# MMAThijssen/catfish

Measured on AMD Instinct MI355X. Metric: signal samples/s classified, higher is better.
Workload: dtype f32

## Files before the change

catfish_amd/csrc/catfish_hip.hip:

```cpp
#include <hip/hip_runtime.h>
#include <stdint.h>
#include <string.h>
#include <stdio.h>
#include <vector>
#include <string>
#include <cmath>
#include <mutex>
#include <set>
#include <functional>

#include "../../include/catfish_hip.h"

typedef float f32x4 __attribute__((ext_vector_type(4)));
typedef float f32x2 __attribute__((ext_vector_type(2)));

#define CF_T 35
#define CF_H 64
#define CF_C 32
#define CF_TILE 16

#define MFMA16(a, b, c) __builtin_amdgcn_mfma_f32_16x16x4f32((a), (b), (c), 0, 0, 0)

#ifndef CF_ABLATE
#define CF_ABLATE 0
#endif
#ifndef CF_PREFETCH
#define CF_PREFETCH 1
#endif

__device__ __forceinline__ float cf_sigmoid(float x) {
    return __builtin_amdgcn_rcpf(1.0f + __expf(-x));
}
__device__ __forceinline__ float cf_tanh(float x) {
    return fmaf(-2.0f, __builtin_amdgcn_rcpf(1.0f + __expf(2.0f * x)), 1.0f);
}
#define CF_GATE_SCALE (-1.4426950408889634)
#define CF_CAND_SCALE (2.8853900817779268)
__device__ __forceinline__ float cf_sigmoid_pre(float a) {
    return __builtin_amdgcn_rcpf(1.0f + __builtin_amdgcn_exp2f(a));
}
__device__ __forceinline__ float cf_tanh_pre(float a) {
    return fmaf(-2.0f, __builtin_amdgcn_rcpf(1.0f + __builtin_amdgcn_exp2f(a)), 1.0f);
}
__device__ __forceinline__ f32x2 cf_sigmoid_pre2(f32x2 a) {
    f32x2 e = {__builtin_amdgcn_exp2f(a.x), __builtin_amdgcn_exp2f(a.y)};
    e = e + (f32x2){1.0f, 1.0f};
    return (f32x2){__builtin_amdgcn_rcpf(e.x), __builtin_amdgcn_rcpf(e.y)};
}
__device__ __forceinline__ f32x2 cf_tanh_pre2(f32x2 a) {
    return __builtin_elementwise_fma((f32x2){-2.0f, -2.0f}, cf_sigmoid_pre2(a), (f32x2){1.0f, 1.0f});
}
template <typename T>
struct far_lds {
    static constexpr int N64K = 65536 / sizeof(T);
    const T *b0, *b1, *b2;
    __device__ __forceinline__ explicit far_lds(const T* base) {
        int o1 = N64K, o2 = 2 * N64K;
        asm volatile("" : "+v"(o1), "+v"(o2));
        b0 = base; b1 = base + o1; b2 = base + o2;
    }
    __device__ __forceinline__ const T& operator[](int e) const { return e < N64K ? b0[e] : (e < 2 * N64K ? b1[e - N64K] : b2[e - 2 * N64K]); }
};
__device__ __forceinline__ f32x4 cf_sigmoid_pre4(f32x4 a) {
    f32x4 e = {__builtin_amdgcn_exp2f(a.x), __builtin_amdgcn_exp2f(a.y), __builtin_amdgcn_exp2f(a.z), __builtin_amdgcn_exp2f(a.w)};
    e = e + (f32x4){1.0f, 1.0f, 1.0f, 1.0f};
    return (f32x4){__builtin_amdgcn_rcpf(e.x), __builtin_amdgcn_rcpf(e.y), __builtin_amdgcn_rcpf(e.z), __builtin_amdgcn_rcpf(e.w)};
}
__device__ __forceinline__ f32x4 cf_tanh_pre4(f32x4 a) {
    return __builtin_elementwise_fma((f32x4){-2.0f, -2.0f, -2.0f, -2.0f}, cf_sigmoid_pre4(a), (f32x4){1.0f, 1.0f, 1.0f, 1.0f});
}
struct cf_dropout {
    float keep_prob = 1.f;
    uint32_t seed = 0;
    int32_t layer = 0;
    const double* step = nullptr;
};
__device__ __forceinline__ uint32_t cf_fmix32(uint32_t v) {
    v ^= v >> 16; v *= 0x85ebca6bu; v ^= v >> 13; v *= 0xc2b2ae35u; v ^= v >> 16;
    return v;
}
__device__ __forceinline__ uint32_t cf_drop_key(const cf_dropout& d) {
    const uint32_t st = d.step ? (uint32_t)(long long)d.step[0] : 0u;
    return cf_fmix32(d.seed ^ cf_fmix32(0x9E3779B9u * (uint32_t)(d.layer + 1) + st * 0x85ebca6bu));
}
__device__ __forceinline__ f32x4 cf_drop_scale4(uint32_t key, float keep_prob, int64_t idx4) {
    const uint32_t thresh = (uint32_t)fminf(keep_prob * 4294967296.0f, 4294967040.0f);
    const float inv = 1.0f / keep_prob;
    const uint64_t e = (uint64_t)idx4 * 4u;
    const uint32_t base = (uint32_t)e ^ ((uint32_t)(e >> 32) * 0x9E3779B9u);
    f32x4 o;
    o.x = cf_fmix32((base + 0u) ^ key) < thresh ? inv : 0.f;
    o.y = cf_fmix32((base + 1u) ^ key) < thresh ? inv : 0.f;
    o.z = cf_fmix32((base + 2u) ^ key) < thresh ? inv : 0.f;
    o.w = cf_fmix32((base + 3u) ^ key) < thresh ? inv : 0.f;
    return o;
}

__device__ __forceinline__ f32x4 relu4(f32x4 v) {
    f32x4 o;
    o.x = fmaxf(v.x, 0.f); o.y = fmaxf(v.y, 0.f); o.z = fmaxf(v.z, 0.f); o.w = fmaxf(v.w, 0.f);
    return o;
}

__host__ __device__ constexpr int gru_x_floats(int cin) { return (cin / 4) * 3 * 256; }
__host__ __device__ constexpr int gru_hg_floats() { return 16 * 2 * 256; }
__host__ __device__ constexpr int gru_hc_floats() { return 16 * 256; }
__host__ __device__ constexpr int gru_bias_off(int cin) { return gru_x_floats(cin) + gru_hg_floats() + gru_hc_floats(); }
__host__ __device__ constexpr int gru_dense_off(int cin) { return gru_bias_off(cin) + 192; }
__host__ __device__ constexpr int gru_pack_floats(int cin) { return gru_dense_off(cin) + 64; }
#include "tuned_launch.hpp"

__host__ __device__ constexpr int res_units(bool first) { return first ? 4 : 6; }
__host__ __device__ constexpr int res_vecs(bool first) { return first ? 6 : 4; }
__host__ __device__ constexpr int res_pack_floats(bool first) { return res_units(first) * 1024 + res_vecs(first) * 32; }

__host__ __device__ constexpr int frag_feature(int ks, int q) { return 16 * (ks >> 2) + 4 * q + (ks & 3); }

__device__ __forceinline__ void unit_mma(const float* __restrict__ unit, int lane, const f32x4 (&in)[2], f32x4 (&acc)[2]) {
    const f32x2* u2 = reinterpret_cast<const f32x2*>(unit) + lane;
#pragma unroll
    for (int ks = 0; ks < 8; ++ks) {
        const f32x2 a = u2[ks * 64];
        const float b = in[ks >> 2][ks & 3];
        acc[0] = MFMA16(a.x, b, acc[0]);
        acc[1] = MFMA16(a.y, b, acc[1]);
    }
}

template <bool FIRST>
__global__ __launch_bounds__(256) void res_block_kernel(const float* __restrict__ wpack,
                                                        const float* __restrict__ x_nat,
                                                        const f32x4* __restrict__ x_frag,
                                                        f32x4* __restrict__ y_frag,
                                                        int64_t n_windows, int n_tiles, int t_chunks) {
    extern __shared__ __attribute__((aligned(16))) float lds[];
    constexpr int PACK = res_pack_floats(FIRST);
    constexpr int VEC0 = res_units(FIRST) * 1024;
    {
        const f32x4* src = reinterpret_cast<const f32x4*>(wpack);
        f32x4* dst = reinterpret_cast<f32x4*>(lds);
        for (int i = threadIdx.x; i < PACK / 4; i += blockDim.x) dst[i] = src[i];
    }
    __syncthreads();
    const int lane = threadIdx.x & 63;
    const int wave = __builtin_amdgcn_readfirstlane(threadIdx.x >> 6);
    const int q = lane >> 4;
    const int waves_per_block = blockDim.x >> 6;
    float* xs = lds + PACK + wave * (CF_TILE * CF_T);

    auto vec = [&](int v, int mo) -> f32x4 {
        return *reinterpret_cast<const f32x4*>(lds + VEC0 + v * 32 + mo * 16 + q * 4);
    };

    const int chunk_len = (CF_T + t_chunks - 1) / t_chunks;
    for (int task = blockIdx.x * waves_per_block + wave; task < n_tiles * t_chunks; task += gridDim.x * waves_per_block) {
        const int tile = task / t_chunks;
        const int p0 = (task - tile * t_chunks) * chunk_len;
        const int p1 = min(p0 + chunk_len, CF_T);
        f32x4 w_sc[2], b_sc[2], w_f[2], b_f[2];
        if constexpr (FIRST) {
            const int64_t base = (int64_t)tile * CF_TILE * CF_T;
            const int64_t limit = n_windows * CF_T;
            for (int i = lane; i < CF_TILE * CF_T; i += 64) xs[i] = (base + i < limit) ? x_nat[base + i] : 0.f;
#pragma unroll
            for (int mo = 0; mo < 2; ++mo) { w_sc[mo] = vec(2, mo); b_sc[mo] = vec(3, mo); w_f[mo] = vec(4, mo); b_f[mo] = vec(5, mo); }
            __builtin_amdgcn_fence(__ATOMIC_RELEASE, "wavefront");
            __builtin_amdgcn_wave_barrier();
            __builtin_amdgcn_fence(__ATOMIC_ACQUIRE, "wavefront");
        }
        f32x4 o1_pp[2] = {{0, 0, 0, 0}, {0, 0, 0, 0}};
        f32x4 o1_p[2] = {{0, 0, 0, 0}, {0, 0, 0, 0}};
        f32x4 sc_p[2] = {{0, 0, 0, 0}, {0, 0, 0, 0}};
        for (int i = p0 > 0 ? p0 - 1 : 0; i <= p1; ++i) {
            f32x4 o1_c[2] = {{0, 0, 0, 0}, {0, 0, 0, 0}};
            f32x4 sc_c[2] = {{0, 0, 0, 0}, {0, 0, 0, 0}};
            if (i < CF_T) {
                if constexpr (FIRST) {
                    const float xv = xs[(lane & 15) * CF_T + i];
#pragma unroll
                    for (int mo = 0; mo < 2; ++mo) {
                        sc_c[mo] = w_sc[mo] * xv + b_sc[mo];
                        o1_c[mo] = relu4(w_f[mo] * xv + b_f[mo]);
                    }
                } else {
                    f32x4 in[2];
                    const f32x4* src = x_frag + ((int64_t)tile * CF_T + i) * 2 * 64 + lane;
                    in[0] = src[0];
                    in[1] = src[64];
                    sc_c[0] = vec(0, 0); sc_c[1] = vec(0, 1);
                    unit_mma(lds + 0 * 1024, lane, in, sc_c);
                    f32x4 acc[2] = {vec(1, 0), vec(1, 1)};
                    unit_mma(lds + 1 * 1024, lane, in, acc);
                    o1_c[0] = relu4(acc[0]); o1_c[1] = relu4(acc[1]);
                }
            }
            if (i >= p0 + 1) {
                constexpr int U3 = FIRST ? 0 : 2;
                constexpr int VB3 = FIRST ? 0 : 2;
                f32x4 acc[2] = {vec(VB3, 0), vec(VB3, 1)};
                unit_mma(lds + (U3 + 0) * 1024, lane, o1_pp, acc);
                unit_mma(lds + (U3 + 1) * 1024, lane, o1_p, acc);
                unit_mma(lds + (U3 + 2) * 1024, lane, o1_c, acc);
                f32x4 o2[2] = {relu4(acc[0]), relu4(acc[1])};
                f32x4 acc3[2] = {vec(VB3 + 1, 0), vec(VB3 + 1, 1)};
                unit_mma(lds + (U3 + 3) * 1024, lane, o2, acc3);
                f32x4* dst = y_frag + ((int64_t)tile * CF_T + (i - 1)) * 2 * 64 + lane;
                dst[0] = relu4(relu4(acc3[0]) + sc_p[0]);
                dst[64] = relu4(relu4(acc3[1]) + sc_p[1]);
            }
#pragma unroll
            for (int mo = 0; mo < 2; ++mo) { o1_pp[mo] = o1_p[mo]; o1_p[mo] = o1_c[mo]; sc_p[mo] = sc_c[mo]; }
        }
        if constexpr (FIRST) __builtin_amdgcn_wave_barrier();
    }
}

template <bool CHUNKED>
__global__ __launch_bounds__(256) void res_stack2_kernel(const float* __restrict__ wpack0, const float* __restrict__ wpack1,
                                                         const float* __restrict__ x_nat,
                                                         f32x4* __restrict__ y_frag,
                                                         f32x4* __restrict__ y0_frag,
                                                         int64_t n_windows, int n_tiles, int t_chunks) {
    extern __shared__ __attribute__((aligned(16))) float lds[];
    constexpr int PACK0 = res_pack_floats(true), PACK1 = res_pack_floats(false);
    constexpr int VEC0 = res_units(true) * 1024, VEC1 = res_units(false) * 1024;
    {
        const f32x4* src0 = reinterpret_cast<const f32x4*>(wpack0);
        const f32x4* src1 = reinterpret_cast<const f32x4*>(wpack1);
        f32x4* dst = reinterpret_cast<f32x4*>(lds);
        for (int i = threadIdx.x; i < PACK0 / 4; i += blockDim.x) dst[i] = src0[i];
        for (int i = threadIdx.x; i < PACK1 / 4; i += blockDim.x) dst[PACK0 / 4 + i] = src1[i];
    }
    __syncthreads();
    const int lane = threadIdx.x & 63;
    const int wave = __builtin_amdgcn_readfirstlane(threadIdx.x >> 6);
    const int q = lane >> 4;
    const int waves_per_block = blockDim.x >> 6;
    const float* w0 = lds;
    const float* w1 = lds + PACK0;
    float* xs = lds + PACK0 + PACK1 + wave * (CF_TILE * CF_T);
    auto vec0 = [&](int v, int mo) -> f32x4 { return *reinterpret_cast<const f32x4*>(w0 + VEC0 + v * 32 + mo * 16 + q * 4); };
    auto vec1 = [&](int v, int mo) -> f32x4 { return *reinterpret_cast<const f32x4*>(w1 + VEC1 + v * 32 + mo * 16 + q * 4); };
    const f32x4 zero = {0, 0, 0, 0};

    if (!CHUNKED) t_chunks = 1;
    const int chunk_len = CHUNKED ? (CF_T + t_chunks - 1) / t_chunks : CF_T;
    for (int task = blockIdx.x * waves_per_block + wave; task < n_tiles * t_chunks; task += gridDim.x * waves_per_block) {
        const int tile = CHUNKED ? task / t_chunks : task;
        const int p0 = CHUNKED ? (task - tile * t_chunks) * chunk_len : 0;
        const int p1 = CHUNKED ? min(p0 + chunk_len, CF_T) : CF_T;
        if (CHUNKED && p0 >= p1) continue;
        {
            const int64_t base = (int64_t)tile * CF_TILE * CF_T;
            const int64_t limit = n_windows * CF_T;
            for (int i = lane; i < CF_TILE * CF_T; i += 64) xs[i] = (base + i < limit) ? x_nat[base + i] : 0.f;
            __builtin_amdgcn_fence(__ATOMIC_RELEASE, "wavefront");
            __builtin_amdgcn_wave_barrier();
            __builtin_amdgcn_fence(__ATOMIC_ACQUIRE, "wavefront");
        }
        f32x4 w_sc[2], b_sc[2], w_f[2], b_f[2];
#pragma unroll
        for (int mo = 0; mo < 2; ++mo) { w_sc[mo] = vec0(2, mo); b_sc[mo] = vec0(3, mo); w_f[mo] = vec0(4, mo); b_f[mo] = vec0(5, mo); }
        f32x4 a_pp[2] = {zero, zero}, a_p[2] = {zero, zero}, a_sp[2] = {zero, zero};
        f32x4 b_pp[2] = {zero, zero}, b_p[2] = {zero, zero}, b_sp[2] = {zero, zero};
        for (int i = p0 > 2 ? p0 - 2 : 0; i <= p1 + 1; ++i) {
            f32x4 a_c[2] = {zero, zero}, a_sc[2] = {zero, zero};
            if (i < CF_T) {
                const float xv = xs[(lane & 15) * CF_T + i];
#pragma unroll
                for (int mo = 0; mo < 2; ++mo) {
                    a_sc[mo] = w_sc[mo] * xv + b_sc[mo];
                    a_c[mo] = relu4(w_f[mo] * xv + b_f[mo]);
                }
            }
            f32x4 y0[2] = {zero, zero};
            const bool have_y0 = i >= 1 && i <= CF_T && i >= p0;
            if (have_y0) {
                f32x4 acc[2] = {vec0(0, 0), vec0(0, 1)};
                unit_mma(w0 + 0 * 1024, lane, a_pp, acc);
                unit_mma(w0 + 1 * 1024, lane, a_p, acc);
                unit_mma(w0 + 2 * 1024, lane, a_c, acc);
                f32x4 o2[2] = {relu4(acc[0]), relu4(acc[1])};
                f32x4 acc3[2] = {vec0(1, 0), vec0(1, 1)};
                unit_mma(w0 + 3 * 1024, lane, o2, acc3);
                y0[0] = relu4(relu4(acc3[0]) + a_sp[0]);
                y0[1] = relu4(relu4(acc3[1]) + a_sp[1]);
                if (CHUNKED && y0_frag && i - 1 >= p0 && i - 1 < p1) {
                    f32x4* d0 = y0_frag + ((int64_t)tile * CF_T + (i - 1)) * 2 * 64 + lane;
                    d0[0] = y0[0];
                    d0[64] = y0[1];
                }
            }
            f32x4 b_c[2] = {zero, zero}, b_sc[2] = {zero, zero};
            if (have_y0) {
                b_sc[0] = vec1(0, 0); b_sc[1] = vec1(0, 1);
                unit_mma(w1 + 0 * 1024, lane, y0, b_sc);
                f32x4 acc[2] = {vec1(1, 0), vec1(1, 1)};
                unit_mma(w1 + 1 * 1024, lane, y0, acc);
                b_c[0] = relu4(acc[0]); b_c[1] = relu4(acc[1]);
            }
            if (i >= 2 && i - 2 >= p0 && i - 2 < p1) {
                f32x4 acc[2] = {vec1(2, 0), vec1(2, 1)};
                unit_mma(w1 + 2 * 1024, lane, b_pp, acc);
                unit_mma(w1 + 3 * 1024, lane, b_p, acc);
                unit_mma(w1 + 4 * 1024, lane, b_c, acc);
                f32x4 o2[2] = {relu4(acc[0]), relu4(acc[1])};
                f32x4 acc3[2] = {vec1(3, 0), vec1(3, 1)};
                unit_mma(w1 + 5 * 1024, lane, o2, acc3);
                f32x4* dst = y_frag + ((int64_t)tile * CF_T + (i - 2)) * 2 * 64 + lane;
                dst[0] = relu4(relu4(acc3[0]) + b_sp[0]);
                dst[64] = relu4(relu4(acc3[1]) + b_sp[1]);
            }
#pragma unroll
            for (int mo = 0; mo < 2; ++mo) {
                a_pp[mo] = a_p[mo]; a_p[mo] = a_c[mo]; a_sp[mo] = a_sc[mo];
                if (i >= 1) { b_pp[mo] = b_p[mo]; b_p[mo] = b_c[mo]; b_sp[mo] = b_sc[mo]; }
            }
        }
        __builtin_amdgcn_wave_barrier();
    }
}

template <int CIN>
__device__ __forceinline__ void gru_stage_weights(float* lds, const float* __restrict__ wpack, int dir) {
    constexpr int PACK = gru_pack_floats(CIN);
    const f32x4* src = reinterpret_cast<const f32x4*>(wpack + (size_t)dir * PACK);
    f32x4* dst = reinterpret_cast<f32x4*>(lds);
    for (int i = threadIdx.x; i < PACK / 4; i += blockDim.x) dst[i] = src[i];
}

#ifndef CF_SCHED_DS_FIRST
#define CF_SCHED_DS_FIRST 1
#endif
#if CF_SCHED_DS_FIRST
#define CF_KSTEP_SCHED(nds, nmfma)                               \
    __builtin_amdgcn_sched_group_barrier(0x100, nds, 0);         \
    __builtin_amdgcn_sched_group_barrier(0x008, nmfma, 0);       \
    __builtin_amdgcn_sched_barrier(0)
#else
#define CF_KSTEP_SCHED(nds, nmfma) __builtin_amdgcn_sched_barrier(0)
#endif
template <int CIN, bool LAST, bool STASH = false, bool SKIP0 = false>
__device__ __forceinline__ void gru_tile(const float* lds, int lane, int dir, int tile, const f32x4* __restrict__ X,
                                         f32x4* __restrict__ Y, float* __restrict__ P, int n_tiles,
                                         f32x4* __restrict__ S = nullptr, f32x4* __restrict__ YD = nullptr, cf_dropout drop = cf_dropout(),
                                         int s_begin = 0, int s_end = CF_T, f32x4* HO = nullptr, bool skip0 = false) {
    const uint32_t drop_key = (STASH && YD) ? cf_drop_key(drop) : 0u;
    constexpr int KGX = CIN / 16;
    constexpr int KSX = CIN / 4;
    constexpr int XN4 = gru_x_floats(CIN) / 4;
    constexpr int HG4 = gru_hg_floats() / 4;
    constexpr int BIAS = gru_bias_off(CIN);
    constexpr int DENSE = gru_dense_off(CIN);
    const int q = lane >> 4;
    const f32x4* WX = reinterpret_cast<const f32x4*>(lds) + lane;
    const far_lds<f32x4> WL(WX);
    const f32x4* B4 = reinterpret_cast<const f32x4*>(lds + BIAS) + q;
    const f32x4* D4 = reinterpret_cast<const f32x4*>(lds + DENSE) + q;
    {
        f32x4 h[4] = {{0, 0, 0, 0}, {0, 0, 0, 0}, {0, 0, 0, 0}, {0, 0, 0, 0}};
        if (s_begin > 0) {
#pragma unroll
            for (int m = 0; m < 4; ++m) h[m] = HO[m * 64 + lane];
        }
        f32x4 xc[KGX];
        {
            const int t0 = dir ? (CF_T - 1 - s_begin) : s_begin;
            const f32x4* src = X + ((int64_t)tile * CF_T + t0) * KGX * 64 + lane;
#pragma unroll
            for (int g = 0; g < KGX; ++g) xc[g] = src[g * 64];
        }
        for (int s = s_begin; s < s_end; ++s) {
            const int t = dir ? (CF_T - 1 - s) : s;
            f32x4 acc[12];
#pragma unroll
            for (int mo = 0; mo < 12; ++mo) acc[mo] = B4[mo * 4];
            constexpr int PF = CF_PREFETCH;
            auto loadA = [&](int p, f32x4 (&d)[3]) {
                if (p < KSX) { d[0] = WL[(p * 3 + 0) * 64]; d[1] = WL[(p * 3 + 1) * 64]; d[2] = WL[(p * 3 + 2) * 64]; }
                else if (p < KSX + 16) { d[0] = WL[XN4 + ((p - KSX) * 2 + 0) * 64]; d[1] = WL[XN4 + ((p - KSX) * 2 + 1) * 64]; }
                else if (p < KSX + 32) { d[0] = WL[XN4 + HG4 + (p - KSX - 16) * 64]; }
            };
            f32x4 ac[3], an[3], a2[3];
            loadA(0, ac);
            if (PF == 2) loadA(1, an);
#pragma unroll
            for (int ks = 0; ks < KSX; ++ks) {
                if (PF == 2) loadA(ks + 2, a2); else loadA(ks + 1, an);
                const float b = xc[ks >> 2][ks & 3];
#pragma unroll
                for (int g = 0; g < 3; ++g) {
                    acc[4 * g + 0] = MFMA16(ac[g].x, b, acc[4 * g + 0]);
                    acc[4 * g + 1] = MFMA16(ac[g].y, b, acc[4 * g + 1]);
                    acc[4 * g + 2] = MFMA16(ac[g].z, b, acc[4 * g + 2]);
                    acc[4 * g + 3] = MFMA16(ac[g].w, b, acc[4 * g + 3]);
                }
                CF_KSTEP_SCHED(3, 12);
#pragma unroll
                for (int g = 0; g < 3; ++g) { ac[g] = an[g]; if (PF == 2) an[g] = a2[g]; }
            }
            {
                int tn = dir ? (t - 1) : (t + 1);
                tn = tn < 0 ? 0 : (tn > CF_T - 1 ? CF_T - 1 : tn);
                const f32x4* src = X + ((int64_t)tile * CF_T + tn) * KGX * 64 + lane;
#pragma unroll
                for (int g = 0; g < KGX; ++g) if (!(CF_ABLATE & 2)) xc[g] = src[g * 64];
            }
            const bool run_h = !SKIP0 || !(skip0 && s == 0);
            if constexpr (SKIP0) {
#pragma unroll
                for (int mo = 0; mo < 12; ++mo) asm volatile("" : "+v"(acc[mo]));
            }
            if (run_h) {
#pragma unroll
            for (int ks = 0; ks < 16; ++ks) {
                if (PF == 2) loadA(KSX + ks + 2, a2); else loadA(KSX + ks + 1, an);
                const float b = h[ks >> 2][ks & 3];
#pragma unroll
                for (int g = 0; g < 2; ++g) {
                    acc[4 * g + 0] = MFMA16(ac[g].x, b, acc[4 * g + 0]);
                    acc[4 * g + 1] = MFMA16(ac[g].y, b, acc[4 * g + 1]);
                    acc[4 * g + 2] = MFMA16(ac[g].z, b, acc[4 * g + 2]);
                    acc[4 * g + 3] = MFMA16(ac[g].w, b, acc[4 * g + 3]);
                }
                CF_KSTEP_SCHED(2, 8);
                ac[0] = an[0]; ac[1] = an[1];
                if (PF == 2) { an[0] = a2[0]; an[1] = a2[1]; }
            }
            f32x4 rh[4];
#pragma unroll
            for (int m = 0; m < 4; ++m) {
                if (CF_ABLATE & 1) { rh[m] = acc[m] * 0.001f; continue; }
                const f32x4 rv = cf_sigmoid_pre4(acc[m]);
                rh[m] = rv * h[m];
                if constexpr (STASH) acc[m] = rv;
            }
#pragma unroll
            for (int ks = 0; ks < 16; ++ks) {
                if (PF == 2) loadA(KSX + 16 + ks + 2, a2); else loadA(KSX + 16 + ks + 1, an);
                const float b = rh[ks >> 2][ks & 3];
                acc[8] = MFMA16(ac[0].x, b, acc[8]);
                acc[9] = MFMA16(ac[0].y, b, acc[9]);
                acc[10] = MFMA16(ac[0].z, b, acc[10]);
                acc[11] = MFMA16(ac[0].w, b, acc[11]);
                CF_KSTEP_SCHED(1, 4);
                ac[0] = an[0];
                if (PF == 2) an[0] = a2[0];
            }
            }
#pragma unroll
            for (int m = 0; m < 4; ++m) {
                if (CF_ABLATE & 1) { h[m] = acc[4 + m] * 0.001f + acc[8 + m] * 0.001f; continue; }
                const f32x4 u = cf_sigmoid_pre4(acc[4 + m]);
                const f32x4 c = cf_tanh_pre4(acc[8 + m]);
                h[m] = __builtin_elementwise_fma(u, h[m] - c, c);
                if constexpr (STASH) { acc[4 + m] = u; acc[8 + m] = c; }
            }
            if constexpr (STASH) {
                f32x4* sdst = S + (((int64_t)tile * CF_T + t) * 2 + dir) * 12 * 64 + lane;
#pragma unroll
                for (int j = 0; j < 12; ++j) sdst[j * 64] = acc[j];
            }
            if constexpr (!LAST) {
                f32x4* dst = Y + (((int64_t)tile * CF_T + t) * 8 + dir * 4) * 64 + lane;
#pragma unroll
                for (int m = 0; m < 4; ++m) if (!(CF_ABLATE & 2) || s == CF_T - 1) dst[m * 64] = h[m];
                if constexpr (STASH) {
                    if (YD) {
                        const int64_t i0 = (((int64_t)tile * CF_T + t) * 8 + dir * 4) * 64 + lane;
#pragma unroll
                        for (int m = 0; m < 4; ++m) YD[i0 + m * 64] = h[m] * cf_drop_scale4(drop_key, drop.keep_prob, i0 + m * 64);
                    }
                }
            } else {
                float pm[4];
#pragma unroll
                for (int m = 0; m < 4; ++m) {
                    const f32x4 wd = D4[m * 4];
                    pm[m] = wd.x * h[m].x;
                    pm[m] = fmaf(wd.y, h[m].y, pm[m]); pm[m] = fmaf(wd.z, h[m].z, pm[m]); pm[m] = fmaf(wd.w, h[m].w, pm[m]);
                }
                float p = ((pm[0] + pm[1]) + pm[2]) + pm[3];
                p += __shfl_xor(p, 16);
                p += __shfl_xor(p, 32);
                if (lane < 16) P[(((int64_t)dir * n_tiles + tile) * CF_T + t) * 16 + lane] = p;
            }
            __builtin_amdgcn_sched_barrier(0);
        }
        if (s_end < CF_T) {
#pragma unroll
            for (int m = 0; m < 4; ++m) HO[m * 64 + lane] = h[m];
        }
    }
}

__device__ __forceinline__ void cf_handoff_publish(unsigned* flag) {
    asm volatile("s_waitcnt vmcnt(0)" ::: "memory");
    __builtin_amdgcn_fence(__ATOMIC_RELEASE, "workgroup");
    asm volatile("s_waitcnt vmcnt(0)" ::: "memory");
    __hip_atomic_store(flag, 1u, __ATOMIC_RELAXED, __HIP_MEMORY_SCOPE_WORKGROUP);
}
__device__ __forceinline__ void cf_handoff_wait(unsigned* flag, int lane, unsigned* err) {
    if (lane == 0) {
        bool ok = false;
        for (int it = 0; it < 1000000 && !ok; ++it) {
            ok = __hip_atomic_load(flag, __ATOMIC_RELAXED, __HIP_MEMORY_SCOPE_WORKGROUP) != 0u;
            if (!ok) __builtin_amdgcn_s_sleep(16);
        }
        if (!ok && err) __hip_atomic_store(err, 1u, __ATOMIC_RELAXED, __HIP_MEMORY_SCOPE_SYSTEM);
    }
    __builtin_amdgcn_fence(__ATOMIC_ACQUIRE, "workgroup");
    asm volatile("s_waitcnt vmcnt(0)" ::: "memory");
}
__device__ __forceinline__ void cf_handoff_publish_agent(unsigned* flag) {
    asm volatile("s_waitcnt vmcnt(0)" ::: "memory");
    __builtin_amdgcn_fence(__ATOMIC_RELEASE, "agent");
    asm volatile("s_waitcnt vmcnt(0)" ::: "memory");
    __hip_atomic_store(flag, 1u, __ATOMIC_RELAXED, __HIP_MEMORY_SCOPE_AGENT);
}
__device__ __forceinline__ void cf_handoff_wait_agent(unsigned* flag, int lane, unsigned* err) {
    if (lane == 0) {
        bool ok = false;
        for (int it = 0; it < 1000000 && !ok; ++it) {
            ok = __hip_atomic_load(flag, __ATOMIC_RELAXED, __HIP_MEMORY_SCOPE_AGENT) != 0u;
            if (!ok) __builtin_amdgcn_s_sleep(16);
        }
        if (!ok && err) __hip_atomic_store(err, 1u, __ATOMIC_RELAXED, __HIP_MEMORY_SCOPE_SYSTEM);
    }
    __builtin_amdgcn_fence(__ATOMIC_ACQUIRE, "agent");
    asm volatile("s_waitcnt vmcnt(0)" ::: "memory");
    if (lane == 0) __hip_atomic_store(flag, 0u, __ATOMIC_RELAXED, __HIP_MEMORY_SCOPE_AGENT);
}


template <int CIN, bool LAST>
__global__ __launch_bounds__(512, 2) void gru_layer_kernel(const float* __restrict__ wpack,
                                                           const f32x4* __restrict__ X,
                                                           f32x4* __restrict__ Y,
                                                           float* __restrict__ P,
                                                           int n_tiles,
                                                           int balance_arg,
                                                           f32x4* hand,
                                                           unsigned* gflags,
                                                           unsigned* err) {
    extern __shared__ __attribute__((aligned(16))) float lds[];
    const int dir = blockIdx.y;
    gru_stage_weights<CIN>(lds, wpack, dir);
    unsigned* flags = reinterpret_cast<unsigned*>(lds + gru_pack_floats(CIN));
    if (threadIdx.x < CF_GRU_MAX_WAVES) flags[threadIdx.x] = 0u;
    __syncthreads();
    const int lane = threadIdx.x & 63;
    const int wave = __builtin_amdgcn_readfirstlane(threadIdx.x >> 6);
    const int nwaves = blockDim.x >> 6;
    const int balance = balance_arg & CF_GRU_SCHED_MASK;
    const bool skip0 = !(balance_arg & CF_GRU_RUN_ZERO_PRODUCTS);
    int t0 = (int)((int64_t)blockIdx.x * n_tiles / gridDim.x);
    const int t1 = (int)((int64_t)(blockIdx.x + 1) * n_tiles / gridDim.x);
    cf_gru_share sh;
    int n_pieces;
    if (balance == 2) {
        sh = cf_gru_balanced_share(n_tiles, (int)gridDim.x * nwaves, (int)blockIdx.x * nwaves + wave, CF_T);
        n_pieces = (sh.head_end > 0) + sh.whole_count + (sh.tail_begin < CF_T);
        t0 = 0;
    } else if (balance) {
        sh = cf_gru_balanced_share(t1 - t0, nwaves, wave, CF_T);
        n_pieces = (sh.head_end > 0) + sh.whole_count + (sh.tail_begin < CF_T);
    } else {
        sh.head_tile = sh.head_end = 0; sh.whole_first = sh.whole_count = 0; sh.tail_tile = 0; sh.tail_begin = CF_T;
        n_pieces = t1 - t0 > wave ? (t1 - t0 - wave + nwaves - 1) / nwaves : 0;
    }
    f32x4* slots = hand + ((size_t)(dir * gridDim.x + blockIdx.x) * CF_GRU_MAX_WAVES) * 4 * 64;
    unsigned* gflag = gflags + dir * gridDim.x + blockIdx.x;
    const int has_head = balance && sh.head_end > 0;
    for (int i = 0; i < n_pieces; ++i) {
        int tile, s_begin = 0, s_end = CF_T;
        f32x4* ho = nullptr;
        if (!balance) {
            tile = t0 + wave + i * nwaves;
        } else if (i < has_head) {
            tile = t0 + sh.head_tile; s_end = sh.head_end; ho = slots + wave * 4 * 64;
        } else if (i < has_head + sh.whole_count) {
            tile = t0 + sh.whole_first + (i - has_head);
        } else {
            tile = t0 + sh.tail_tile; s_begin = sh.tail_begin;
            if (wave > 0) {
                ho = slots + (wave - 1) * 4 * 64;
                cf_handoff_wait(flags + (wave - 1), lane, err);
            } else {
                ho = slots - (CF_GRU_MAX_WAVES - (nwaves - 1)) * 4 * 64;
                cf_handoff_wait_agent(gflag - 1, lane, err);
            }
        }
        gru_tile<CIN, LAST, false, true>(lds, lane, dir, tile, X, Y, P, n_tiles, nullptr, nullptr, cf_dropout(), s_begin, s_end, ho, skip0);
        if (s_end < CF_T) {
            if (wave < nwaves - 1) cf_handoff_publish(flags + wave);
            else cf_handoff_publish_agent(gflag);
        }
    }
}

struct cf_fused_args {
    const float* w[3];
    const f32x4* x0;
    f32x4* y[2];
    float* p;
    unsigned* flags;
    int lds_floats;
    unsigned* err;
    int n_tiles;
    int groups;
    int n_layers;
    int cin0;
};

__device__ __forceinline__ bool cf_wait_flag(unsigned* flag) {
    for (int it = 0; it < 1000000; ++it) {
        if (__hip_atomic_load(flag, __ATOMIC_RELAXED, __HIP_MEMORY_SCOPE_AGENT) != 0u) return true;
        __builtin_amdgcn_s_sleep(16);
    }
    return false;
}

template <int CIN, bool LAST>
__device__ __forceinline__ void gru_fused_worker(float* lds, const cf_fused_args& a, int layer, int dir) {
// ... 1850 lines not shown
```

Measured before the change: 344.6 million.

## Unroll res_stack2 time loop by three with register rotation and batch staging loads

Rewrites the res_stack2 time loop as a three-step unrolled macro that rotates history registers by name, so per-step copies go away. A fast path drops the boundary checks for interior steps. Weight staging and the per-tile input load now issue several global loads before any LDS stores, raising memory-level parallelism. Adds launch_bounds(256,2), which caps register use to allow at least two blocks, at the cost of larger code and possible spills.

```diff
diff --git a/catfish_amd/csrc/catfish_hip.hip b/catfish_amd/csrc/catfish_hip.hip
--- a/catfish_amd/csrc/catfish_hip.hip
+++ b/catfish_amd/csrc/catfish_hip.hip
@@ -100,6 +100,20 @@
     f32x4 o;
     o.x = fmaxf(v.x, 0.f); o.y = fmaxf(v.y, 0.f); o.z = fmaxf(v.z, 0.f); o.w = fmaxf(v.w, 0.f);
     return o;
+}
+template <int NB>
+__device__ __forceinline__ void cf_stage_copy(f32x4* dst, const f32x4* __restrict__ src, int n4) {
+    const int stride = blockDim.x;
+    for (int base = threadIdx.x; base < n4; base += NB * stride) {
+        f32x4 v[NB];
+#pragma unroll
+        for (int k = 0; k < NB; ++k) v[k] = src[min(base + k * stride, n4 - 1)];
+#pragma unroll
+        for (int k = 0; k < NB; ++k) asm volatile("" : "+v"(v[k]));
+#pragma unroll
+        for (int k = 0; k < NB; ++k)
+            if (base + k * stride < n4) dst[base + k * stride] = v[k];
+    }
 }
 
 __host__ __device__ constexpr int gru_x_floats(int cin) { return (cin / 4) * 3 * 256; }
@@ -215,8 +229,57 @@
     }
 }
 
+#define CF_RES2_STEP(full, i, a_pp, a_p, a_c, a_sp, a_sc, b_pp, b_p, b_c, b_sp, b_sc) do { \
+    const int ql = ln >> 4;                                                                \
+    if (full || i < CF_T) {                                                                \
+        const float xv = xs[(ln & 15) * CF_T + i];                                         \
+        _Pragma("unroll")                                                                  \
+        for (int mo = 0; mo < 2; ++mo) {                                                   \
+            a_sc[mo] = w_sc[mo] * xv + b_sc0[mo];                                          \
+            a_c[mo] = relu4(w_f[mo] * xv + b_f[mo]);                                       \
+        }                                                                                  \
+    } else {                                                                               \
+        a_c[0] = zero; a_c[1] = zero; a_sc[0] = zero; a_sc[1] = zero;                      \
+    }                                                                                      \
+    if (full || (i >= 1 && i <= CF_T && i >= p0)) {                                        \
+        f32x4 acc[2] = {vec0(0, 0, ql), vec0(0, 1, ql)};                                   \
+        unit_mma(w0 + 0 * 1024, ln, a_pp, acc);                                            \
+        unit_mma(w0 + 1 * 1024, ln, a_p, acc);                                             \
+        unit_mma(w0 + 2 * 1024, ln, a_c, acc);                                             \
+        f32x4 o2[2] = {relu4(acc[0]), relu4(acc[1])};                                      \
+        f32x4 acc3[2] = {vec0(1, 0, ql), vec0(1, 1, ql)};                                  \
+        unit_mma(w0 + 3 * 1024, ln, o2, acc3);                                             \
+        f32x4 y0[2];                                                                       \
+        y0[0] = relu4(relu4(acc3[0]) + a_sp[0]);                                           \
+        y0[1] = relu4(relu4(acc3[1]) + a_sp[1]);                                           \
+        if (CHUNKED && y0_frag && i - 1 >= p0 && i - 1 < p1) {                             \
+            f32x4* d0 = y0_frag + ((int64_t)tile * CF_T + (i - 1)) * 2 * 64 + ln;          \
+            d0[0] = y0[0];                                                                 \
+            d0[64] = y0[1];                                                                \
+        }                                                                                  \
+        b_sc[0] = vec1(0, 0, ql); b_sc[1] = vec1(0, 1, ql);                                \
+        unit_mma(w1 + 0 * 1024, ln, y0, b_sc);                                             \
+        f32x4 acc1[2] = {vec1(1, 0, ql), vec1(1, 1, ql)};                                  \
+        unit_mma(w1 + 1 * 1024, ln, y0, acc1);                                             \
+        b_c[0] = relu4(acc1[0]); b_c[1] = relu4(acc1[1]);                                  \
+    } else {                                                                               \
+        b_c[0] = zero; b_c[1] = zero; b_sc[0] = zero; b_sc[1] = zero;                      \
+    }                                                                                      \
+    if (full || (i >= 2 && i - 2 >= p0 && i - 2 < p1)) {                                   \
+        f32x4 acc[2] = {vec1(2, 0, ql), vec1(2, 1, ql)};                                   \
+        unit_mma(w1 + 2 * 1024, ln, b_pp, acc);                                            \
+        unit_mma(w1 + 3 * 1024, ln, b_p, acc);                                             \
+        unit_mma(w1 + 4 * 1024, ln, b_c, acc);                                             \
+        f32x4 o2[2] = {relu4(acc[0]), relu4(acc[1])};                                      \
+        f32x4 acc3[2] = {vec1(3, 0, ql), vec1(3, 1, ql)};                                  \
+        unit_mma(w1 + 5 * 1024, ln, o2, acc3);                                             \
+        f32x4* dst = y_frag + ((int64_t)tile * CF_T + (i - 2)) * 2 * 64 + ln;              \
+        dst[0] = relu4(relu4(acc3[0]) + b_sp[0]);                                          \
+        dst[64] = relu4(relu4(acc3[1]) + b_sp[1]);                                         \
+    }                                                                                      \
+} while (0)
 template <bool CHUNKED>
-__global__ __launch_bounds__(256) void res_stack2_kernel(const float* __restrict__ wpack0, const float* __restrict__ wpack1,
+__global__ __launch_bounds__(256, 2) void res_stack2_kernel(const float* __restrict__ wpack0, const float* __restrict__ wpack1,
                                                          const float* __restrict__ x_nat,
                                                          f32x4* __restrict__ y_frag,
                                                          f32x4* __restrict__ y0_frag,
@@ -225,11 +288,9 @@
     constexpr int PACK0 = res_pack_floats(true), PACK1 = res_pack_floats(false);
     constexpr int VEC0 = res_units(true) * 1024, VEC1 = res_units(false) * 1024;
     {
-        const f32x4* src0 = reinterpret_cast<const f32x4*>(wpack0);
-        const f32x4* src1 = reinterpret_cast<const f32x4*>(wpack1);
         f32x4* dst = reinterpret_cast<f32x4*>(lds);
-        for (int i = threadIdx.x; i < PACK0 / 4; i += blockDim.x) dst[i] = src0[i];
-        for (int i = threadIdx.x; i < PACK1 / 4; i += blockDim.x) dst[PACK0 / 4 + i] = src1[i];
+        cf_stage_copy<7>(dst, reinterpret_cast<const f32x4*>(wpack0), PACK0 / 4);
+        cf_stage_copy<7>(dst + PACK0 / 4, reinterpret_cast<const f32x4*>(wpack1), PACK1 / 4);
     }
     __syncthreads();
     const int lane = threadIdx.x & 63;
@@ -239,8 +300,8 @@
     const float* w0 = lds;
     const float* w1 = lds + PACK0;
     float* xs = lds + PACK0 + PACK1 + wave * (CF_TILE * CF_T);
-    auto vec0 = [&](int v, int mo) -> f32x4 { return *reinterpret_cast<const f32x4*>(w0 + VEC0 + v * 32 + mo * 16 + q * 4); };
-    auto vec1 = [&](int v, int mo) -> f32x4 { return *reinterpret_cast<const f32x4*>(w1 + VEC1 + v * 32 + mo * 16 + q * 4); };
+    auto vec0 = [&](int v, int mo, int ql) -> f32x4 { return *reinterpret_cast<const f32x4*>(w0 + VEC0 + v * 32 + mo * 16 + ql * 4); };
+    auto vec1 = [&](int v, int mo, int ql) -> f32x4 { return *reinterpret_cast<const f32x4*>(w1 + VEC1 + v * 32 + mo * 16 + ql * 4); };
     const f32x4 zero = {0, 0, 0, 0};
 
     if (!CHUNKED) t_chunks = 1;
@@ -253,73 +314,53 @@
         {
             const int64_t base = (int64_t)tile * CF_TILE * CF_T;
             const int64_t limit = n_windows * CF_T;
-            for (int i = lane; i < CF_TILE * CF_T; i += 64) xs[i] = (base + i < limit) ? x_nat[base + i] : 0.f;
+            constexpr int XR = (CF_TILE * CF_T + 63) / 64;
+            float xv[XR];
+#pragma unroll
+            for (int k = 0; k < XR; ++k) {
+                const int64_t g = base + min(lane + k * 64, CF_TILE * CF_T - 1);
+                const float v = x_nat[min(g, limit - 1)];
+                xv[k] = g < limit ? v : 0.f;
+            }
+#pragma unroll
+            for (int k = 0; k < XR; ++k) asm volatile("" : "+v"(xv[k]));
+#pragma unroll
+            for (int k = 0; k < XR; ++k)
+                if (lane + k * 64 < CF_TILE * CF_T) xs[lane + k * 64] = xv[k];
             __builtin_amdgcn_fence(__ATOMIC_RELEASE, "wavefront");
             __builtin_amdgcn_wave_barrier();
             __builtin_amdgcn_fence(__ATOMIC_ACQUIRE, "wavefront");
         }
-        f32x4 w_sc[2], b_sc[2], w_f[2], b_f[2];
-#pragma unroll
-        for (int mo = 0; mo < 2; ++mo) { w_sc[mo] = vec0(2, mo); b_sc[mo] = vec0(3, mo); w_f[mo] = vec0(4, mo); b_f[mo] = vec0(5, mo); }
-        f32x4 a_pp[2] = {zero, zero}, a_p[2] = {zero, zero}, a_sp[2] = {zero, zero};
-        f32x4 b_pp[2] = {zero, zero}, b_p[2] = {zero, zero}, b_sp[2] = {zero, zero};
-        for (int i = p0 > 2 ? p0 - 2 : 0; i <= p1 + 1; ++i) {
-            f32x4 a_c[2] = {zero, zero}, a_sc[2] = {zero, zero};
-            if (i < CF_T) {
-                const float xv = xs[(lane & 15) * CF_T + i];
-#pragma unroll
-                for (int mo = 0; mo < 2; ++mo) {
-                    a_sc[mo] = w_sc[mo] * xv + b_sc[mo];
-                    a_c[mo] = relu4(w_f[mo] * xv + b_f[mo]);
-                }
+        f32x4 w_sc[2], b_sc0[2], w_f[2], b_f[2];
+#pragma unroll
+        for (int mo = 0; mo < 2; ++mo) { w_sc[mo] = vec0(2, mo, q); b_sc0[mo] = vec0(3, mo, q); w_f[mo] = vec0(4, mo, q); b_f[mo] = vec0(5, mo, q); }
+        f32x4 a0[2] = {zero, zero}, a1[2] = {zero, zero}, a2[2] = {zero, zero}, as0[2] = {zero, zero}, as1[2], as2[2];
+        f32x4 b0[2] = {zero, zero}, b1[2] = {zero, zero}, b2[2] = {zero, zero}, bs0[2] = {zero, zero}, bs1[2], bs2[2];
+        const int i_end = p1 + 1;
+        const int full_lo = p0 + 2, full_hi = min(CF_T - 1, p1 + 1);
+        for (int i = p0 > 2 ? p0 - 2 : 0; i <= i_end; ++i) {
+            int ln = lane;
+            asm volatile("" : "+v"(ln));
+            if (i >= full_lo && i + 2 <= full_hi) {
+                CF_RES2_STEP(true, i, a0, a1, a2, as0, as1, b0, b1, b2, bs0, bs1);
+                ++i;
+                asm volatile("" : "+v"(ln));
+                CF_RES2_STEP(true, i, a1, a2, a0, as1, as2, b1, b2, b0, bs1, bs2);
+                ++i;
+                asm volatile("" : "+v"(ln));
+                CF_RES2_STEP(true, i, a2, a0, a1, as2, as0, b2, b0, b1, bs2, bs0);
+            } else {
+                CF_RES2_STEP(false, i, a0, a1, a2, as0, as1, b0, b1, b2, bs0, bs1);
+                if (++i > i_end) break;
+                CF_RES2_STEP(false, i, a1, a2, a0, as1, as2, b1, b2, b0, bs1, bs2);
+                if (++i > i_end) break;
+                CF_RES2_STEP(false, i, a2, a0, a1, as2, as0, b2, b0, b1, bs2, bs0);
             }
-            f32x4 y0[2] = {zero, zero};
-            const bool have_y0 = i >= 1 && i <= CF_T && i >= p0;
-            if (have_y0) {
-                f32x4 acc[2] = {vec0(0, 0), vec0(0, 1)};
-                unit_mma(w0 + 0 * 1024, lane, a_pp, acc);
-                unit_mma(w0 + 1 * 1024, lane, a_p, acc);
-                unit_mma(w0 + 2 * 1024, lane, a_c, acc);
-                f32x4 o2[2] = {relu4(acc[0]), relu4(acc[1])};
-                f32x4 acc3[2] = {vec0(1, 0), vec0(1, 1)};
-                unit_mma(w0 + 3 * 1024, lane, o2, acc3);
-                y0[0] = relu4(relu4(acc3[0]) + a_sp[0]);
-                y0[1] = relu4(relu4(acc3[1]) + a_sp[1]);
-                if (CHUNKED && y0_frag && i - 1 >= p0 && i - 1 < p1) {
-                    f32x4* d0 = y0_frag + ((int64_t)tile * CF_T + (i - 1)) * 2 * 64 + lane;
-                    d0[0] = y0[0];
-                    d0[64] = y0[1];
-                }
-            }
-            f32x4 b_c[2] = {zero, zero}, b_sc[2] = {zero, zero};
-            if (have_y0) {
-                b_sc[0] = vec1(0, 0); b_sc[1] = vec1(0, 1);
-                unit_mma(w1 + 0 * 1024, lane, y0, b_sc);
-                f32x4 acc[2] = {vec1(1, 0), vec1(1, 1)};
-                unit_mma(w1 + 1 * 1024, lane, y0, acc);
-                b_c[0] = relu4(acc[0]); b_c[1] = relu4(acc[1]);
-            }
-            if (i >= 2 && i - 2 >= p0 && i - 2 < p1) {
-                f32x4 acc[2] = {vec1(2, 0), vec1(2, 1)};
-                unit_mma(w1 + 2 * 1024, lane, b_pp, acc);
-                unit_mma(w1 + 3 * 1024, lane, b_p, acc);
-                unit_mma(w1 + 4 * 1024, lane, b_c, acc);
-                f32x4 o2[2] = {relu4(acc[0]), relu4(acc[1])};
-                f32x4 acc3[2] = {vec1(3, 0), vec1(3, 1)};
-                unit_mma(w1 + 5 * 1024, lane, o2, acc3);
-                f32x4* dst = y_frag + ((int64_t)tile * CF_T + (i - 2)) * 2 * 64 + lane;
-                dst[0] = relu4(relu4(acc3[0]) + b_sp[0]);
-                dst[64] = relu4(relu4(acc3[1]) + b_sp[1]);
-            }
-#pragma unroll
-            for (int mo = 0; mo < 2; ++mo) {
-                a_pp[mo] = a_p[mo]; a_p[mo] = a_c[mo]; a_sp[mo] = a_sc[mo];
-                if (i >= 1) { b_pp[mo] = b_p[mo]; b_p[mo] = b_c[mo]; b_sp[mo] = b_sc[mo]; }
-            }
         }
         __builtin_amdgcn_wave_barrier();
     }
 }
+#undef CF_RES2_STEP
 
 template <int CIN>
 __device__ __forceinline__ void gru_stage_weights(float* lds, const float* __restrict__ wpack, int dir) {
```

Result: no change. 345.3 million, median of 6 (+0.2%).
